# yanyan-li/PlanarSLAM

Measured on NVIDIA H100. Metric: rgbd_frames_per_sec_640x480, higher is better.
Workload: dtype u8/f64

## Files before the change

planarslam_b200/csrc/lsd_kernels.cuh:

```cuda
#pragma once
#include <cuda_runtime.h>

#include <cfloat>
#include <cstdint>

#include "lsd_detsincos.h"
#include "lsd_rectenum.h"
#include "pslam_internal.h"

namespace pslam {

struct LsdGeom {
    int w, h;
    int W, H;
    int refine;
    int seg_cap;
    int cand_cap;
    int rect_enum;
    int min_reg_size;
    double rho, prec, p, log_nt, density_th, log_eps;
    const double* lgamma_tab;
};
#define LSD_LGAMMA_N 8192

#define LSD_ANG_UNDEF 0x7f800000u
#define LSD_ANG_USED 0x80000000u

#define LSD_PI 3.14159265358979323846
#define LSD_DEG2RAD (LSD_PI / 180)
#define LSD_3_2_PI ((3 * LSD_PI) / 2)
#define LSD_2PI (2 * LSD_PI)
#define LSD_LN10 2.30258509299404568402

__device__ __forceinline__ float lsd_fast_atan2_deg(float y, float x) {
    const float p1 = 0.9997878412794807f * (float)(180 / 3.14159265358979323846);
    const float p3 = -0.3258083974640975f * (float)(180 / 3.14159265358979323846);
    const float p5 = 0.1555786518463281f * (float)(180 / 3.14159265358979323846);
    const float p7 = -0.04432655554792128f * (float)(180 / 3.14159265358979323846);
    const float ax = fabsf(x), ay = fabsf(y);
    const bool wide = ax >= ay;
    const float num = wide ? ay : ax, den = __fadd_rn(wide ? ax : ay, (float)DBL_EPSILON);
    const float c = __fdiv_rn(num, den);
    const float c2 = __fmul_rn(c, c);
    float a = __fmul_rn(__fadd_rn(__fmul_rn(__fadd_rn(__fmul_rn(__fadd_rn(__fmul_rn(p7, c2), p5), c2), p3), c2), p1), c);
    if (!wide) a = __fsub_rn(90.f, a);
    if (x < 0) a = __fsub_rn(180.f, a);
    if (y < 0) a = __fsub_rn(360.f, a);
    return a;
}
__device__ __forceinline__ double lsd_angle(int gx, int gy) { return (double)lsd_fast_atan2_deg((float)gx, (float)(-gy)) * LSD_DEG2RAD; }
__device__ __forceinline__ double lsd_norm(int gx, int gy) { return sqrt((double)(gx * gx + gy * gy) / 4.0); }

template <int V>
__device__ __noinline__ void lsd_sincos(double x, double& s, double& c) { lsd_sincos_body(x, s, c); }

#define LSD_TW 64
#define LSD_TH 16
#define LSD_SW 88
#define LSD_SH 28
__global__ void __launch_bounds__(256) k_lsd_blur_scale(LsdGeom g, const uint8_t* __restrict__ gray, const int16_t* __restrict__ ix,
                                                        const int16_t* __restrict__ ax, const int16_t* __restrict__ iy, const int16_t* __restrict__ ay,
                                                        uint8_t* __restrict__ scaled) {
    __shared__ uint8_t s_src[LSD_SH][LSD_SW];
    __shared__ uint16_t s_h[LSD_SH][LSD_SW];
    __shared__ uint8_t s_b[LSD_SH][LSD_SW];
    const int frame = blockIdx.z, X0 = blockIdx.x * LSD_TW, Y0 = blockIdx.y * LSD_TH;
    const int X1 = min(X0 + LSD_TW, g.W) - 1, Y1 = min(Y0 + LSD_TH, g.H) - 1;
    const int bx0 = ix[X0], bx1 = min(ix[X1] + 1, g.w - 1), by0 = iy[Y0], by1 = min(iy[Y1] + 1, g.h - 1);
    const int sx0 = bx0 - 2, sy0 = by0 - 2, sw = bx1 - bx0 + 5, sh = by1 - by0 + 5;
    const uint8_t* src = gray + (size_t)frame * g.w * g.h;
    const int lane = threadIdx.x & 31, wid = threadIdx.x >> 5;
    for (int r = wid; r < sh; r += 8) {
        int y = sy0 + r;
        y = y < 0 ? -y : (y >= g.h ? 2 * (g.h - 1) - y : y);
        const uint8_t* srow = src + (size_t)y * g.w;
        for (int c = lane; c < sw; c += 32) {
            int x = sx0 + c;
            x = x < 0 ? -x : (x >= g.w ? 2 * (g.w - 1) - x : x);
            s_src[r][c] = srow[x];
        }
    }
    __syncthreads();
    const int bw = bx1 - bx0 + 1, bh = by1 - by0 + 1;
    for (int r = wid; r < sh; r += 8)
// ... 51 lines not shown
    const int W4 = g.W >> 2;
    const int xq = blockIdx.x * 64 + (threadIdx.x & 63), y = blockIdx.y * 4 + (threadIdx.x >> 6);
    const bool inside = xq < W4 && y < g.H;
    const uint8_t* s = scaled + (size_t)frame * g.W * g.H;
    uint32_t a_w[4] = {LSD_ANG_UNDEF, LSD_ANG_UNDEF, LSD_ANG_UNDEF, LSD_ANG_UNDEF}, g_w[4] = {0, 0, 0, 0};
    float2 cs[4];
#pragma unroll
    for (int i = 0; i < 4; ++i) cs[i] = make_float2(0.f, 0.f);
    int sq = 0;
    if (inside && y < g.H - 1) {
        const int x = xq * 4;
        const uint32_t* r0 = reinterpret_cast<const uint32_t*>(s + (size_t)y * g.W + x);
        const uint32_t* r1 = reinterpret_cast<const uint32_t*>(s + (size_t)(y + 1) * g.W + x);
        const uint32_t w0 = r0[0], w1 = r1[0];
        const bool more = x + 4 < g.W;
        const uint32_t n0 = more ? (uint32_t)s[(size_t)y * g.W + x + 4] : 0u, n1 = more ? (uint32_t)s[(size_t)(y + 1) * g.W + x + 4] : 0u;
        const uint32_t e0 = __funnelshift_r(w0, n0, 8), e1 = __funnelshift_r(w1, n1, 8);
#pragma unroll
        for (int i = 0; i < 4; ++i) {
            if (x + i >= g.W - 1) continue;
            const int pa = (w0 >> (8 * i)) & 255, pb = (e0 >> (8 * i)) & 255, pc = (w1 >> (8 * i)) & 255, pd = (e1 >> (8 * i)) & 255;
            const int DA = pd - pa, BC = pb - pc;
            const int gx = DA + BC, gy = DA - BC;
            g_w[i] = ((uint32_t)gx & 0xffffu) | ((uint32_t)gy << 16);
            if (lsd_norm(gx, gy) > g.rho) {
                sq = max(sq, gx * gx + gy * gy); a_w[i] = __float_as_uint(lsd_fast_atan2_deg((float)gx, (float)(-gy)));
                cs[i] = __ldg(cs_lut + (gx + 510) * 1021 + (gy + 510));
            }
        }
    }
    if (inside) {
        const size_t o = (size_t)frame * g.W * g.H + (size_t)y * g.W + (size_t)xq * 4;
        *reinterpret_cast<uint4*>(ang + o) = make_uint4(a_w[0], a_w[1], a_w[2], a_w[3]);
        *reinterpret_cast<uint4*>(gxy + o) = make_uint4(g_w[0], g_w[1], g_w[2], g_w[3]);
        float4* co = reinterpret_cast<float4*>(cs_out + o);
        co[0] = make_float4(cs[0].x, cs[0].y, cs[1].x, cs[1].y);
        co[1] = make_float4(cs[2].x, cs[2].y, cs[3].x, cs[3].y);
    }
    for (int o = 16; o; o >>= 1) sq = max(sq, __shfl_xor_sync(0xffffffffu, sq, o));
    if ((threadIdx.x & 31) == 0 && sq > 0) atomicMax(&smax[frame], sq);
}

struct LsdRect { double x1, y1, x2, y2, width, x, y, theta, dx, dy, prec, p; };

#define LSD_RING 64
struct LsdFrame {
    uint32_t* ang;
    const float2* cs; const uint32_t* gxy;
    uint32_t* reg; uint32_t* order;
    int W, H;
};
__device__ __forceinline__ bool lsd_word_used(uint32_t w) { return (w & LSD_ANG_USED) != 0; }
__device__ __forceinline__ bool lsd_word_defined(uint32_t w) { return (w & 0x7fffffffu) < LSD_ANG_UNDEF; }
__device__ __forceinline__ float lsd_word_deg(uint32_t w) { return __uint_as_float(w & 0x7fffffffu); }
__device__ __forceinline__ double lsd_word_angle(uint32_t w) { return (double)lsd_word_deg(w) * LSD_DEG2RAD; }
__device__ __forceinline__ double lsd_pix_norm(const LsdFrame& F, int x, int y) {
    const uint32_t v = __ldg(F.gxy + (size_t)y * F.W + x);
    return lsd_norm((int)(short)(v & 0xffff), (int)(short)(v >> 16));
}

__device__ __forceinline__ bool lsd_aligned_angle(double a, double theta, double prec) {
    double n_theta = theta - a;
    if (n_theta < 0) n_theta = -n_theta;
    if (n_theta > LSD_3_2_PI) {
        n_theta -= LSD_2PI;
        if (n_theta < 0) n_theta = -n_theta;
    }
    return n_theta <= prec;
}

__device__ __forceinline__ double lsd_angle_diff_signed(double a, double b) {
    double diff = a - b;
    while (diff <= -LSD_PI) diff += LSD_2PI;
    while (diff > LSD_PI) diff -= LSD_2PI;
    return diff;
}
__device__ __forceinline__ bool lsd_double_equal(double a, double b) {
    if (a == b) return true;
    const double abs_diff = fabs(a - b), aa = fabs(a), bb = fabs(b);
    double abs_max = (aa > bb) ? aa : bb;
    if (abs_max < DBL_MIN) abs_max = DBL_MIN;
    return (abs_diff / abs_max) <= (100.0 * DBL_EPSILON);
}
__device__ __forceinline__ double lsd_dist_sq(double x1, double y1, double x2, double y2) { return (x2 - x1) * (x2 - x1) + (y2 - y1) * (y2 - y1); }

struct LsdGrown { double angle; int size; };
template <int V>
__device__ __noinline__ LsdGrown lsd_region_grow(uint32_t* ang, const float2* __restrict__ cs, uint32_t* reg, int W, int H, uint32_t seed, double prec) {
    __shared__ uint32_t ring[LSD_RING];
    const int lane = threadIdx.x & 31;
    const unsigned below = (1u << lane) - 1u;
    const int q = lane >> 3, k8 = lane & 7;
    const int kk = k8 + (k8 >= 4);
    const int dyl = kk / 3 - 1, dxl = kk % 3 - 1;
    const int sx = seed & 0xffff, sy = seed >> 16;
    const uint32_t ws = ang[(size_t)sy * W + sx];
    double reg_angle = lsd_word_angle(ws);
    float sumdx = 0.f, sumdy = 0.f;
    if (lane == 0) { reg[0] = seed; ring[0] = seed; ang[(size_t)sy * W + sx] = ws | LSD_ANG_USED; }
    __syncwarp();
    auto probe = [&](int idx, int size, uint32_t& npix, uint32_t& w, float2& csv) {
        const uint32_t pp = size - idx <= LSD_RING ? ring[idx & (LSD_RING - 1)] : reg[idx];
        const int nx = (int)(pp & 0xffff) + dxl, ny = (int)(pp >> 16) + dyl;
        if (nx >= 0 && ny >= 0 && nx < W && ny < H) {
            const size_t o = (size_t)ny * W + nx;
            w = ang[o]; csv = __ldg(cs + o); npix = (uint32_t)nx | ((uint32_t)ny << 16);
        }
    };
    int size = 1, i = 0;
    bool have_next = false;
    uint32_t np_next = 0xffffffffu, w_next = LSD_ANG_UNDEF;
    float2 cs_next = make_float2(0.f, 0.f);
    while (true) {
        const int navail = min(4, size - i);
        uint32_t npix = 0xffffffffu, w = LSD_ANG_UNDEF;
        float2 csv = make_float2(0.f, 0.f);
        if (have_next) { npix = np_next; w = w_next; csv = cs_next; }
        else if (q < navail) probe(i + q, size, npix, w, csv);
        have_next = size - i >= 8;
        np_next = 0xffffffffu; w_next = LSD_ANG_UNDEF; cs_next = make_float2(0.f, 0.f);
        if (have_next) probe(i + 4 + q, size, np_next, w_next, cs_next);
// ... 180 lines not shown
            const bool hole = idx < m && far_point(reg[idx]);
            const unsigned h = __ballot_sync(0xffffffffu, hole);
            if (hole) reg[idx] = reg[size - 1 - (r + __popc(h & below))];
            r += __popc(h);
        }
        __syncwarp();
        size = m;
        if (size < 2) return false;
        lsd_region2rect<V>(F, size, reg_angle, g.prec, g.p, rec);
        density = lsd_density(size, rec);
    }
    return true;
}

__device__ __forceinline__ double lsd_log_gamma1(double x) {
    if (x > 15.0) return 0.918938533204673 + (x - 0.5) * log(x) - x + 0.5 * x * log(x * sinh(1 / x) + 1 / (810.0 * pow(x, 6.0)));
    const double q[7] = {75122.6331530, 80916.6278952, 36308.2951477, 8687.24529705, 1168.92649479, 83.8676043424, 2.50662827511};
    double a = (x + 0.5) * log(x + 5.5) - (x + 5.5);
    double b = 0;
    for (int n = 0; n < 7; ++n) {
        a -= log(x + (double)n);
        b += q[n] * pow(x, (double)n);
    }
    return a + log(b);
}
__device__ __noinline__ double lsd_nfa_scalar(int n, int k, double p, double log_nt, const double* __restrict__ lgamma_tab) {
    if (n == 0 || k == 0) return -log_nt;
    if (n == k) return -log_nt - (double)n * log10(p);
    const double p_term = p / (1 - p);
    double lg0, lg1, lg2;
    if (n + 1 < LSD_LGAMMA_N) { lg0 = __ldg(lgamma_tab + n + 1); lg1 = __ldg(lgamma_tab + k + 1); lg2 = __ldg(lgamma_tab + n - k + 1); }
    else { lg0 = lsd_log_gamma1((double)n + 1); lg1 = lsd_log_gamma1((double)k + 1); lg2 = lsd_log_gamma1((double)(n - k) + 1); }
    const double log1term = lg0 - lg1 - lg2 + (double)k * log(p) + (double)(n - k) * log(1.0 - p);
    double term = exp(log1term);
    if (lsd_double_equal(term, 0)) {
        if (k > n * p) return -log1term / LSD_LN10 - log_nt;
        return -log_nt;
    }
    double bin_tail = term;
    const double tolerance = 0.1;
    for (int i = k + 1; i <= n; ++i) {
        const double bin_term = (double)(n - i + 1) / (double)i;
        const double mult_term = bin_term * p_term;
        term *= mult_term;
        bin_tail += term;
        if (bin_term < 1) {
            const double err = term * ((1 - pow(mult_term, (double)(n - i + 1))) / (1 - mult_term) - 1);
            if (err < tolerance * fabs(-log10(bin_tail) - log_nt) * bin_tail) break;
        }
    }
    return -log10(bin_tail) - log_nt;
}

__device__ __forceinline__ double lsd_inter_low(double x, double x1, double y1, double x2, double y2) {
    if (lsd_double_equal(x1, x2) && y1 < y2) return y1;
    if (lsd_double_equal(x1, x2) && y1 > y2) return y2;
    return y1 + (x - x1) * (y2 - y1) / (x2 - x1);
}
__device__ __forceinline__ double lsd_inter_hi(double x, double x1, double y1, double x2, double y2) {
    if (lsd_double_equal(x1, x2) && y1 < y2) return y2;
    if (lsd_double_equal(x1, x2) && y1 > y2) return y1;
    return y1 + (x - x1) * (y2 - y1) / (x2 - x1);
}

__device__ __forceinline__ void lsd_rect_count(const LsdFrame& F, const LsdGeom& g, const LsdRect& r, int sub, int stride, int& n, int& k) {
    double vx[4], vy[4], rx[4], ry[4];
    vx[0] = r.x1 - r.dy * r.width / 2.0; vy[0] = r.y1 + r.dx * r.width / 2.0;
    vx[1] = r.x2 - r.dy * r.width / 2.0; vy[1] = r.y2 + r.dx * r.width / 2.0;
    vx[2] = r.x2 + r.dy * r.width / 2.0; vy[2] = r.y2 - r.dx * r.width / 2.0;
    vx[3] = r.x1 + r.dy * r.width / 2.0; vy[3] = r.y1 - r.dx * r.width / 2.0;
    int offset;
    if (r.x1 < r.x2 && r.y1 <= r.y2) offset = 0;
    else if (r.x1 >= r.x2 && r.y1 < r.y2) offset = 1;
    else if (r.x1 > r.x2 && r.y1 >= r.y2) offset = 2;
    else offset = 3;
#pragma unroll
    for (int q = 0; q < 4; ++q) { rx[q] = vx[(offset + q) & 3]; ry[q] = vy[(offset + q) & 3]; }
    n = 0; k = 0;
    const int xa = (int)ceil(rx[0]), xb = (int)floor(rx[2]);
    for (int x = xa + sub; x <= xb; x += stride) {
        if (x < 0 || x >= F.W) continue;
        const double ys = (double)x < rx[3] ? lsd_inter_low(x, rx[0], ry[0], rx[3], ry[3]) : lsd_inter_low(x, rx[3], ry[3], rx[2], ry[2]);
        const double ye = (double)x < rx[1] ? lsd_inter_hi(x, rx[0], ry[0], rx[1], ry[1]) : lsd_inter_hi(x, rx[1], ry[1], rx[2], ry[2]);
        for (int y = (int)ceil(ys); (double)y <= ye; ++y) {
            if (y < 0 || y >= F.H) continue;
            ++n;
            const uint32_t wq = __ldg(F.ang + (size_t)y * F.W + x);
            if (lsd_word_defined(wq) && lsd_aligned_angle(lsd_word_angle(wq), r.theta, r.prec)) ++k;
        }
    }
}

__device__ __forceinline__ void lsd_rect_count_cv4(const LsdFrame& F, const LsdGeom& g, const LsdRect& r, int& n, int& k) {
    LsdRowScan S;
    lsd_cv4_setup(r.x1, r.y1, r.x2, r.y2, r.width, r.dx, r.dy, S);
    n = 0; k = 0;
    const int ya = S.y0 < 0 ? 0 : S.y0, yb = S.c2 < F.H - 1 ? S.c2 : F.H - 1;
    for (int y = ya; y <= yb; ++y) {
        int xa, xb;
        lsd_cv4_row(S, y, xa, xb);
        if (xa < 0) xa = 0;
        if (xb > F.W - 1) xb = F.W - 1;
        for (int x = xa; x <= xb; ++x) {
            ++n;
            const uint32_t wq = __ldg(F.ang + (size_t)y * F.W + x);
            if (lsd_word_defined(wq) && lsd_aligned_angle(lsd_word_angle(wq), r.theta, r.prec)) ++k;
        }
    }
}

__device__ __forceinline__ double lsd_rect_nfa_scalar(const LsdFrame& F, const LsdGeom& g, const LsdRect& r) {
    int n, k;
    if (g.rect_enum == 1) lsd_rect_count_cv4(F, g, r, n, k);
    else lsd_rect_count(F, g, r, 0, 1, n, k);
    return lsd_nfa_scalar(n, k, r.p, g.log_nt, g.lgamma_tab);
}
__device__ __forceinline__ void lsd_rect_count_cv4_prec5(const LsdFrame& F, const LsdRect& r, const double prec[5], int& n, int k[5]) {
    LsdRowScan S;
    lsd_cv4_setup(r.x1, r.y1, r.x2, r.y2, r.width, r.dx, r.dy, S);
    n = 0;
#pragma unroll
    for (int j = 0; j < 5; ++j) k[j] = 0;
    const int ya = S.y0 < 0 ? 0 : S.y0, yb = S.c2 < F.H - 1 ? S.c2 : F.H - 1;
    for (int y = ya; y <= yb; ++y) {
        int xa, xb;
        lsd_cv4_row(S, y, xa, xb);
        if (xa < 0) xa = 0;
        if (xb > F.W - 1) xb = F.W - 1;
        for (int x = xa; x <= xb; ++x) {
            ++n;
            const uint32_t wq = __ldg(F.ang + (size_t)y * F.W + x);
            if (!lsd_word_defined(wq)) continue;
            double n_theta = r.theta - lsd_word_angle(wq);
            if (n_theta < 0) n_theta = -n_theta;
            if (n_theta > LSD_3_2_PI) { n_theta -= LSD_2PI; if (n_theta < 0) n_theta = -n_theta; }
#pragma unroll
            for (int j = 0; j < 5; ++j) k[j] += n_theta <= prec[j];
        }
    }
}
__device__ __noinline__ double lsd_rect_improve_rest(const LsdFrame& F, const LsdGeom& g, LsdRect& rec, double log_nfa) {
    const double delta = 0.5, delta_2 = delta / 2.0;
    for (int stage = 0; stage < 5; ++stage) {
        LsdRect r = rec;
        if ((stage == 0 || stage == 4) && g.rect_enum == 1) {
            if (stage == 0 || (r.width - delta) >= 0.5) {
                double pv[5], precv[5];
                int nn, kk[5];
                double pp = r.p;
#pragma unroll
                for (int n = 0; n < 5; ++n) { pp /= 2; pv[n] = pp; precv[n] = pp * LSD_PI; }
                lsd_rect_count_cv4_prec5(F, r, precv, nn, kk);
#pragma unroll
                for (int n = 0; n < 5; ++n) {
                    r.p = pv[n]; r.prec = precv[n];
                    const double v = lsd_nfa_scalar(nn, kk[n], r.p, g.log_nt, g.lgamma_tab);
                    if (v > log_nfa) { log_nfa = v; rec = r; }
                }
            }
            if (stage < 4 && log_nfa > g.log_eps) return log_nfa;
            continue;
        }
        for (int n = 0; n < 5; ++n) {
            if (stage == 0) { r.p /= 2; r.prec = r.p * LSD_PI; }
            else {
                if (!((r.width - delta) >= 0.5)) continue;
                if (stage == 1) r.width -= delta;
                else if (stage == 2) { r.x1 += -r.dy * delta_2; r.y1 += r.dx * delta_2; r.x2 += -r.dy * delta_2; r.y2 += r.dx * delta_2; r.width -= delta; }
                else if (stage == 3) { r.x1 -= -r.dy * delta_2; r.y1 -= r.dx * delta_2; r.x2 -= -r.dy * delta_2; r.y2 -= r.dx * delta_2; r.width -= delta; }
                else { r.p /= 2; r.prec = r.p * LSD_PI; }
            }
            const double v = lsd_rect_nfa_scalar(F, g, r);
            if (v > log_nfa) { log_nfa = v; rec = r; }
        }
        if (stage < 4 && log_nfa > g.log_eps) return log_nfa;
    }
    return log_nfa;
}

#define LSD_ORDER_THREADS 1024
#define LSD_ORDER_SMEM (32 * 1024 * 4)
__device__ __forceinline__ int lsd_order_bin(const uint8_t* __restrict__ s, int W, int x, int y, double rho, double bin_coef) {
    const size_t a = (size_t)y * W + x;
    const int DA = (int)s[a + W + 1] - (int)s[a], BC = (int)s[a + 1] - (int)s[a + W];
    const int gx = DA + BC, gy = DA - BC;
    const double nrm = lsd_norm(gx, gy);
    return nrm > rho ? (int)(nrm * bin_coef) : -1;
}
__global__ void __launch_bounds__(LSD_ORDER_THREADS) k_lsd_order(LsdGeom g, const uint8_t* __restrict__ scaled, const int32_t* __restrict__ smax,
                                                                uint32_t* __restrict__ order_all, int32_t* __restrict__ n_order) {
    extern __shared__ uint32_t s_cnt[];
    __shared__ uint32_t s_tot[1024];
    __shared__ uint32_t s_wsum[32];
    const int frame = blockIdx.x, tid = threadIdx.x, lane = tid & 31, wid = tid >> 5;
    const int sm = smax[frame];
    if (sm <= 0) { if (tid == 0) n_order[frame] = 0; return; }
    const size_t npx = (size_t)g.W * g.H;
    const uint8_t* s = scaled + (size_t)frame * npx;
    uint32_t* order = order_all + (size_t)frame * npx;
    const double max_grad = sqrt((double)sm / 4.0);
    const double bin_coef = (double)(1024 - 1) / max_grad;
    for (int t = tid; t < 32 * 1024; t += LSD_ORDER_THREADS) s_cnt[t] = 0;
    __syncthreads();
    const int Wm = g.W - 1, n_scan = Wm * (g.H - 1);
    const int per = ((n_scan + 31) / 32 + 31) & ~31;
    const int t0 = wid * per, t1 = min(n_scan, t0 + per);
    uint32_t* cnt = s_cnt + wid * 1024;
    for (int base = t0; base < t1; base += 32) {
        const int t = base + lane;
        int bin = -1;
        if (t < t1) { const int y = t / Wm, x = t - y * Wm; bin = lsd_order_bin(s, g.W, x, y, g.rho, bin_coef); }
        const unsigned peers = __match_any_sync(0xffffffffu, bin);
        if (bin >= 0 && lane == __ffs(peers) - 1) cnt[bin] += __popc(peers);
        __syncwarp();
    }
    __syncthreads();
    {
        const int rb = 1023 - tid;
        uint32_t tot = 0;
        for (int w = 0; w < 32; ++w) tot += s_cnt[w * 1024 + rb];
        uint32_t incl = tot;
        for (int o = 1; o < 32; o <<= 1) { const uint32_t v = __shfl_up_sync(0xffffffffu, incl, o); if (lane >= o) incl += v; }
        if (lane == 31) s_wsum[wid] = incl;
        __syncthreads();
        if (wid == 0) {
// ... 37 lines not shown
    LsdFrame F;
    F.ang = ang_all + (size_t)frame * npx; F.cs = cs_all + (size_t)frame * npx; F.gxy = gxy_all + (size_t)frame * npx; F.reg = reg_all + (size_t)frame * npx;
    F.order = const_cast<uint32_t*>(order_all) + (size_t)frame * npx; F.W = g.W; F.H = g.H;
    int count_out = 0;
    const int n_def = smax[frame] > 0 ? n_order[frame] : 0;
    {
        for (int base = 0; base < n_def; base += 32) {
            const uint32_t mypix = base + lane < n_def ? F.order[base + lane] : 0u;
            int last = -1;
            while (true) {
                bool fresh = false;
                if (base + lane < n_def && lane > last) fresh = !lsd_word_used(F.ang[(size_t)(mypix >> 16) * F.W + (mypix & 0xffff)]);
                const unsigned m = __ballot_sync(0xffffffffu, fresh);
                if (!m) break;
                const int j = __ffs(m) - 1;
                last = j;
                const uint32_t seed = __shfl_sync(0xffffffffu, mypix, j);
                const LsdGrown gr = lsd_region_grow<V>(F.ang, F.cs, F.reg, F.W, F.H, seed, g.prec);
                int size = gr.size;
                double reg_angle = gr.angle;
                if (size < g.min_reg_size) continue;
                LsdRect rc;
                lsd_region2rect<V>(F, size, reg_angle, g.prec, g.p, rc);
                if (g.refine > 0 && !lsd_refine<V>(F, g, size, reg_angle, rc)) continue;
                if (count_out < g.cand_cap && lane < 12) {
                    const double v = lane == 0 ? rc.x1 : lane == 1 ? rc.y1 : lane == 2 ? rc.x2 : lane == 3 ? rc.y2 : lane == 4 ? rc.width : lane == 5 ? rc.x :
                                     lane == 6 ? rc.y : lane == 7 ? rc.theta : lane == 8 ? rc.dx : lane == 9 ? rc.dy : lane == 10 ? rc.prec : rc.p;
                    cands[((size_t)frame * g.cand_cap + count_out) * 12 + lane] = v;
                }
                ++count_out;
            }
        }
    }
    if (lane == 0) {
        n_cand[frame] = count_out;
        status[frame] = count_out > g.cand_cap ? 1 : 0;
    }
}

__device__ __forceinline__ void lsd_load_cand(const double* __restrict__ c, LsdRect& rc) {
    rc.x1 = c[0]; rc.y1 = c[1]; rc.x2 = c[2]; rc.y2 = c[3]; rc.width = c[4]; rc.x = c[5]; rc.y = c[6]; rc.theta = c[7]; rc.dx = c[8]; rc.dy = c[9];
    rc.prec = c[10]; rc.p = c[11];
}
__global__ void __launch_bounds__(64) k_lsd_validate(LsdGeom g, const uint32_t* __restrict__ ang_all, const double* __restrict__ cands, const int32_t* __restrict__ n_cand,
                                                     double* __restrict__ cand_nfa, uint32_t* __restrict__ fail_list, int32_t* __restrict__ n_fail) {
    const int frame = blockIdx.y;
    const int ci = blockIdx.x * 64 + threadIdx.x;
    const int n = min(n_cand[frame], g.cand_cap);
    if (ci >= n) return;
    LsdFrame F;
    F.ang = const_cast<uint32_t*>(ang_all) + (size_t)frame * g.W * g.H; F.cs = nullptr; F.gxy = nullptr; F.reg = nullptr; F.order = nullptr; F.W = g.W; F.H = g.H;
    LsdRect rc;
    lsd_load_cand(cands + ((size_t)frame * g.cand_cap + ci) * 12, rc);
    const double log_nfa = lsd_rect_nfa_scalar(F, g, rc);
    cand_nfa[(size_t)frame * g.cand_cap + ci] = log_nfa;
    if (!(log_nfa > g.log_eps)) fail_list[(size_t)frame * g.cand_cap + atomicAdd(&n_fail[frame], 1)] = (uint32_t)ci;
}
__global__ void __launch_bounds__(64) k_lsd_improve(LsdGeom g, const uint32_t* __restrict__ ang_all, double* __restrict__ cands, double* __restrict__ cand_nfa,
                                                    const uint32_t* __restrict__ fail_list, const int32_t* __restrict__ n_fail) {
    const int frame = blockIdx.y;
    const int k = blockIdx.x * 64 + threadIdx.x;
    if (k >= n_fail[frame]) return;
    const int ci = (int)fail_list[(size_t)frame * g.cand_cap + k];
    LsdFrame F;
    F.ang = const_cast<uint32_t*>(ang_all) + (size_t)frame * g.W * g.H; F.cs = nullptr; F.gxy = nullptr; F.reg = nullptr; F.order = nullptr; F.W = g.W; F.H = g.H;
    double* c = cands + ((size_t)frame * g.cand_cap + ci) * 12;
    LsdRect rc;
    lsd_load_cand(c, rc);
    const double log_nfa = lsd_rect_improve_rest(F, g, rc, cand_nfa[(size_t)frame * g.cand_cap + ci]);
    c[0] = rc.x1; c[1] = rc.y1; c[2] = rc.x2; c[3] = rc.y2; c[4] = rc.width; c[11] = rc.p;
    cand_nfa[(size_t)frame * g.cand_cap + ci] = log_nfa;
}

__global__ void __launch_bounds__(256) k_lsd_emit(LsdGeom g, const double* __restrict__ cands, const int32_t* __restrict__ n_cand, const double* __restrict__ cand_nfa,
                                                  float4* __restrict__ segs, double* __restrict__ wpn, int32_t* __restrict__ n_segs, int32_t* __restrict__ status) {
    __shared__ int s_warp[8];
    __shared__ int s_base;
    const int frame = blockIdx.x, tid = threadIdx.x, lane = tid & 31, wid = tid >> 5;
    const int n = min(n_cand[frame], g.cand_cap);
    if (tid == 0) s_base = 0;
    __syncthreads();
    for (int c0 = 0; c0 < n; c0 += 256) {
        const int ci = c0 + tid;
        bool keep = false;
        double nfa = -1;
        if (ci < n) {
            if (g.refine >= 2) { nfa = cand_nfa[(size_t)frame * g.cand_cap + ci]; keep = nfa > g.log_eps; }
            else keep = true;
        }
        const unsigned m = __ballot_sync(0xffffffffu, keep);
        if (lane == 0) s_warp[wid] = __popc(m);
        __syncthreads();
        int off = s_base;
        for (int w = 0; w < wid; ++w) off += s_warp[w];
        const int slot = off + __popc(m & ((1u << lane) - 1u));
        if (keep && slot < g.seg_cap) {
            const double* c = cands + ((size_t)frame * g.cand_cap + ci) * 12;
            double x1 = c[0], y1 = c[1], x2 = c[2], y2 = c[3], width = c[4];
            x1 += 0.5; y1 += 0.5; x2 += 0.5; y2 += 0.5;
            x1 /= 0.8; y1 /= 0.8; x2 /= 0.8; y2 /= 0.8; width /= 0.8;
            segs[(size_t)frame * g.seg_cap + slot] = make_float4((float)x1, (float)y1, (float)x2, (float)y2);
            double* o = wpn + ((size_t)frame * g.seg_cap + slot) * 3;
            o[0] = width; o[1] = c[11]; o[2] = nfa;
        }
        __syncthreads();
        if (tid == 0) { int t = 0; for (int w = 0; w < 8; ++w) t += s_warp[w]; s_base += t; }
        __syncthreads();
// ... 63 lines not shown
```

planarslam_b200/csrc/lsd_pipeline.cu:

```cuda
#include <algorithm>
#include <cfloat>
#include <cmath>
#include <cstring>
#include <cstdlib>
#include <string>

#include "lsd_kernels.cuh"
#include "lbd_kernels.cuh"

namespace pslam {

struct LsdBuffers {
    LsdGeom g;
    int max_batch = 0, last_n = 0, max_lines_cap = 0;
    int16_t *d_ix = nullptr, *d_ax = nullptr, *d_iy = nullptr, *d_ay = nullptr;
    float2* d_lut = nullptr; double* d_lgamma = nullptr;
    uint8_t* d_gray = nullptr;
    uint8_t* d_scaled = nullptr; uint32_t* d_ang = nullptr; float2* d_cs = nullptr; uint32_t* d_gxy = nullptr; int32_t* d_smax = nullptr;
    uint32_t* d_reg = nullptr; uint32_t* d_order = nullptr; int32_t* d_norder = nullptr;
    double* d_cands = nullptr; double* d_cand_nfa = nullptr; int32_t* d_ncand = nullptr;
    uint32_t* d_fail = nullptr; int32_t* d_nfail = nullptr;
    float4* d_segs = nullptr; double* d_wpn = nullptr; int32_t* d_nsegs = nullptr; int32_t* d_status = nullptr;
    LsdKeyLine* d_kl = nullptr; double* d_lf = nullptr; int32_t* d_nkl = nullptr;
    int16_t *d_dx = nullptr, *d_dy = nullptr; float *d_glocal = nullptr, *d_gglobal = nullptr; uint8_t* d_ldesc = nullptr; float* d_lbd72 = nullptr;
    std::vector<int32_t> h_n, h_status;
};

static int lsd_cv_round(double v) { return (int)std::nearbyint(v); }

static float host_fast_atan2_deg(float y, float x) {
    const float p1 = 0.9997878412794807f * (float)(180 / 3.14159265358979323846);
    const float p3 = -0.3258083974640975f * (float)(180 / 3.14159265358979323846);
    const float p5 = 0.1555786518463281f * (float)(180 / 3.14159265358979323846);
    const float p7 = -0.04432655554792128f * (float)(180 / 3.14159265358979323846);
    const float ax = std::fabs(x), ay = std::fabs(y);
    float a, c, c2;
    if (ax >= ay) { c = ay / (ax + (float)DBL_EPSILON); c2 = c * c; a = (((p7 * c2 + p5) * c2 + p3) * c2 + p1) * c; }
    else { c = ax / (ay + (float)DBL_EPSILON); c2 = c * c; a = 90.f - (((p7 * c2 + p5) * c2 + p3) * c2 + p1) * c; }
    if (x < 0) a = 180.f - a;
    if (y < 0) a = 360.f - a;
    return a;
}

static const int LSD_SEG_CAP = 4096;
#define LSD_REGIONS_OCC 24

int lsd_alloc(pslam_ctx* c) {
    if (c->lsd) return PSLAM_OK;
    LsdBuffers* Bp = new LsdBuffers();
    LsdBuffers& B = *Bp;
    LsdGeom& g = B.g;
    g.w = c->cfg.width; g.h = c->cfg.height;
    const double SCALE = 0.8, ANG_TH = 22.5, QUANT = 2.0;
    g.W = lsd_cv_round(g.w * SCALE); g.H = lsd_cv_round(g.h * SCALE);
    if (g.W < 8 || g.H < 8 || g.W > 32767 || g.H > 32767) { delete Bp; return set_error(c, PSLAM_E_INVALID, "image size unsupported by the line-segment detector"); }
    g.refine = 2;
    g.seg_cap = g.cand_cap = std::max(LSD_SEG_CAP, (int)(((long long)LSD_SEG_CAP * g.w * g.h / (640 * 480) + 1023) / 1024 * 1024));
    {
        const char* e = std::getenv("PSLAM_LSD_RECT_ENUM");
        g.rect_enum = (e && (!std::strcmp(e, "published") || !std::strcmp(e, "0"))) ? 0 : 1;
    }
    g.prec = LSD_PI * ANG_TH / 180; g.p = ANG_TH / 180; g.rho = QUANT / std::sin(g.prec);
    g.log_nt = 5 * (std::log10(double(g.W)) + std::log10(double(g.H))) / 2 + std::log10(11.0);
    g.min_reg_size = (int)(size_t)(-g.log_nt / std::log10(g.p));
    g.density_th = 0.7; g.log_eps = 0;
    B.max_batch = c->cfg.max_batch;
    auto coef = [SCALE](int dn, int sn, std::vector<int16_t>& idx, std::vector<int16_t>& a) {
        idx.resize(dn); a.resize(dn);
        const double scale = 1.0 / SCALE;
        for (int d = 0; d < dn; ++d) {
            const double f = (d + 0.5) * scale - 0.5;
            int i = (int)std::floor(f);
            double fr = f - i;
            if (i < 0) { i = 0; fr = 0; }
            if (i >= sn - 1) { i = sn - 1; fr = 0; }
            idx[d] = (int16_t)i; a[d] = (int16_t)std::floor(fr * 256 + 0.5);
        }
    };
    std::vector<int16_t> ix, ax, iy, ay;
    coef(g.W, g.w, ix, ax); coef(g.H, g.h, iy, ay);
    for (int X0 = 0; X0 < g.W; X0 += LSD_TW) {
        const int X1 = std::min(X0 + LSD_TW, g.W) - 1;
        if (std::min(ix[X1] + 1, g.w - 1) - ix[X0] + 5 > LSD_SW) { delete Bp; return set_error(c, PSLAM_E_INVALID, "LSD tile bound (width)"); }
    }
    for (int Y0 = 0; Y0 < g.H; Y0 += LSD_TH) {
        const int Y1 = std::min(Y0 + LSD_TH, g.H) - 1;
        if (std::min(iy[Y1] + 1, g.h - 1) - iy[Y0] + 5 > LSD_SH) { delete Bp; return set_error(c, PSLAM_E_INVALID, "LSD tile bound (height)"); }
    }
    std::vector<float2> lut((size_t)1021 * 1021);
    for (int gx = -510; gx <= 510; ++gx)
        for (int gy = -510; gy <= 510; ++gy) {
            const double ang = (double)host_fast_atan2_deg((float)gx, (float)(-gy)) * LSD_DEG2RAD;
            const float af = (float)ang;
            lut[(size_t)(gx + 510) * 1021 + (gy + 510)] = make_float2(std::cos(af), std::sin(af));
        }
    std::vector<double> lgam(LSD_LGAMMA_N, 0.0);
    for (int i = 1; i < LSD_LGAMMA_N; ++i) {
        const double x = (double)i;
        if (x > 15.0) lgam[i] = 0.918938533204673 + (x - 0.5) * std::log(x) - x + 0.5 * x * std::log(x * std::sinh(1 / x) + 1 / (810.0 * std::pow(x, 6.0)));
        else {
            static const double q[7] = {75122.6331530, 80916.6278952, 36308.2951477, 8687.24529705, 1168.92649479, 83.8676043424, 2.50662827511};
            double a = (x + 0.5) * std::log(x + 5.5) - (x + 5.5), b = 0;
            for (int n = 0; n < 7; ++n) { a -= std::log(x + double(n)); b += q[n] * std::pow(x, double(n)); }
            lgam[i] = a + std::log(b);
        }
    }
    const size_t npx = (size_t)g.W * g.H, nb = (size_t)B.max_batch;
#define LA(ptr, bytes) do { const int rc_ = check_cuda(c, cudaMalloc((void**)&(ptr), (bytes)), "cudaMalloc(lsd)"); if (rc_ != PSLAM_OK) { c->lsd = Bp; lsd_free(c); return rc_; } } while (0)
    LA(B.d_ix, g.W * 2); LA(B.d_ax, g.W * 2); LA(B.d_iy, g.H * 2); LA(B.d_ay, g.H * 2); LA(B.d_lut, lut.size() * sizeof(float2)); LA(B.d_lgamma, LSD_LGAMMA_N * 8);
    LA(B.d_gray, nb * g.w * g.h); LA(B.d_scaled, nb * npx); LA(B.d_ang, nb * npx * 4); LA(B.d_cs, nb * npx * 8); LA(B.d_gxy, nb * npx * 4); LA(B.d_smax, nb * 4);
    LA(B.d_reg, nb * npx * 4); LA(B.d_order, nb * npx * 4); LA(B.d_norder, nb * 4);
    LA(B.d_fail, nb * g.cand_cap * 4); LA(B.d_nfail, nb * 4);
    LA(B.d_cands, nb * g.cand_cap * 12 * 8); LA(B.d_cand_nfa, nb * g.cand_cap * 8); LA(B.d_ncand, nb * 4);
    LA(B.d_segs, nb * g.seg_cap * sizeof(float4)); LA(B.d_wpn, nb * g.seg_cap * 3 * 8); LA(B.d_nsegs, nb * 4); LA(B.d_status, nb * 4);
#undef LA
    cudaStream_t st = c->stream;
    PSLAM_CUDA(c, cudaMemcpyAsync(B.d_ix, ix.data(), g.W * 2, cudaMemcpyHostToDevice, st));
    PSLAM_CUDA(c, cudaMemcpyAsync(B.d_ax, ax.data(), g.W * 2, cudaMemcpyHostToDevice, st));
    PSLAM_CUDA(c, cudaMemcpyAsync(B.d_iy, iy.data(), g.H * 2, cudaMemcpyHostToDevice, st));
    PSLAM_CUDA(c, cudaMemcpyAsync(B.d_ay, ay.data(), g.H * 2, cudaMemcpyHostToDevice, st));
    PSLAM_CUDA(c, cudaMemcpyAsync(B.d_lut, lut.data(), lut.size() * sizeof(float2), cudaMemcpyHostToDevice, st));
    PSLAM_CUDA(c, cudaMemcpyAsync(B.d_lgamma, lgam.data(), LSD_LGAMMA_N * 8, cudaMemcpyHostToDevice, st));
    g.lgamma_tab = B.d_lgamma;
    PSLAM_CUDA(c, cudaStreamSynchronize(st));
    c->lsd = Bp;
    return PSLAM_OK;
}

void lsd_free(pslam_ctx* c) {
    if (!c->lsd) return;
    LsdBuffers& B = *c->lsd;
    for (void* p : {(void*)B.d_ix, (void*)B.d_ax, (void*)B.d_iy, (void*)B.d_ay, (void*)B.d_lut, (void*)B.d_lgamma, (void*)B.d_gray, (void*)B.d_scaled, (void*)B.d_ang, (void*)B.d_cs, (void*)B.d_gxy,
                    (void*)B.d_smax, (void*)B.d_reg, (void*)B.d_order, (void*)B.d_norder, (void*)B.d_segs, (void*)B.d_wpn,
                    (void*)B.d_nsegs, (void*)B.d_status, (void*)B.d_cands, (void*)B.d_cand_nfa, (void*)B.d_ncand, (void*)B.d_fail, (void*)B.d_nfail, (void*)B.d_kl, (void*)B.d_lf, (void*)B.d_nkl, (void*)B.d_dx, (void*)B.d_dy, (void*)B.d_glocal, (void*)B.d_gglobal,
                    (void*)B.d_ldesc, (void*)B.d_lbd72})
        if (p) cudaFree(p);
    delete c->lsd;
    c->lsd = nullptr;
}

int lsd_detect_dev(pslam_ctx* c, const uint8_t* d_gray, int nframes, int refine) {
    int rc = lsd_alloc(c);
    if (rc != PSLAM_OK) return rc;
    LsdBuffers& B = *c->lsd;
    if (nframes < 1 || nframes > B.max_batch) return set_error(c, PSLAM_E_INVALID, "nframes outside [1, max_batch]");
    if (refine < 0 || refine > 2) return set_error(c, PSLAM_E_INVALID, "refine must be 0, 1 or 2");
    LsdGeom g = B.g;
    g.refine = refine;
    cudaStream_t st = c->stream;
    const size_t npx = (size_t)g.W * g.H;
    PSLAM_CUDA(c, cudaMemsetAsync(B.d_smax, 0, (size_t)nframes * 4, st));
    const dim3 gb((g.W + LSD_TW - 1) / LSD_TW, (g.H + LSD_TH - 1) / LSD_TH, nframes);
    PSLAM_LAUNCH(c, "lsd_blur_scale", k_lsd_blur_scale<<<gb, 256, 0, st>>>(g, d_gray, B.d_ix, B.d_ax, B.d_iy, B.d_ay, B.d_scaled));
    if ((g.W & 3) == 0 && !std::getenv("PSLAM_LSD_GRADIENT1")) {
        const dim3 gg4(((g.W >> 2) + 63) / 64, (g.H + 3) / 4, nframes);
        PSLAM_LAUNCH(c, "lsd_gradient", k_lsd_gradient4<<<gg4, 256, 0, st>>>(g, B.d_scaled, B.d_lut, B.d_ang, B.d_cs, B.d_gxy, B.d_smax));
    } else {
        const dim3 gg((g.W + 63) / 64, (g.H + 3) / 4, nframes);
        PSLAM_LAUNCH(c, "lsd_gradient", k_lsd_gradient<<<gg, 256, 0, st>>>(g, B.d_scaled, B.d_lut, B.d_ang, B.d_cs, B.d_gxy, B.d_smax));
    }
    PSLAM_CUDA(c, cudaFuncSetAttribute(k_lsd_order, cudaFuncAttributeMaxDynamicSharedMemorySize, LSD_ORDER_SMEM));
    if ((size_t)B.g.seg_cap * sizeof(float) > 48 * 1024) {
        if ((size_t)B.g.seg_cap * sizeof(float) > 227 * 1024) return set_error(c, PSLAM_E_INVALID, "image too large for the key-line ranking buffer");
        PSLAM_CUDA(c, cudaFuncSetAttribute(k_lsd_keylines, cudaFuncAttributeMaxDynamicSharedMemorySize, (int)(B.g.seg_cap * sizeof(float))));
    }
    PSLAM_LAUNCH(c, "lsd_order", k_lsd_order<<<nframes, LSD_ORDER_THREADS, LSD_ORDER_SMEM, st>>>(g, B.d_scaled, B.d_smax, B.d_order, B.d_norder));
    {
        static const int occ = [] { const char* e = std::getenv("PSLAM_LSD_OCC"); const int v = e ? std::atoi(e) : LSD_REGIONS_OCC; return v == 16 || v == 20 || v == 24 || v == 32 ? v : LSD_REGIONS_OCC; }();
#define LSD_REGIONS_LAUNCH(V) PSLAM_LAUNCH(c, "lsd_regions", k_lsd_regions<V><<<nframes, 32, 0, st>>>(g, nframes, B.d_ang, B.d_cs, B.d_gxy, B.d_smax, B.d_reg, B.d_order, B.d_norder, \
                                                                                                B.d_cands, B.d_ncand, B.d_status))
        if (occ == 16) LSD_REGIONS_LAUNCH(16); else if (occ == 20) LSD_REGIONS_LAUNCH(20); else if (occ == 24) LSD_REGIONS_LAUNCH(24); else LSD_REGIONS_LAUNCH(32);
#undef LSD_REGIONS_LAUNCH
    }
    if (refine >= 2) {
        const dim3 gv((g.cand_cap + 63) / 64, nframes);
        PSLAM_CUDA(c, cudaMemsetAsync(B.d_nfail, 0, (size_t)nframes * 4, st));
        PSLAM_LAUNCH(c, "lsd_validate", k_lsd_validate<<<gv, 64, 0, st>>>(g, B.d_ang, B.d_cands, B.d_ncand, B.d_cand_nfa, B.d_fail, B.d_nfail));
        PSLAM_LAUNCH(c, "lsd_improve", k_lsd_improve<<<gv, 64, 0, st>>>(g, B.d_ang, B.d_cands, B.d_cand_nfa, B.d_fail, B.d_nfail));
    }
    PSLAM_LAUNCH(c, "lsd_emit", k_lsd_emit<<<nframes, 256, 0, st>>>(g, B.d_cands, B.d_ncand, B.d_cand_nfa, B.d_segs, B.d_wpn, B.d_nsegs, B.d_status));
    PSLAM_CUDA(c, cudaGetLastError());
    B.last_n = nframes;
    return PSLAM_OK;
}

// ... 195 lines not shown
```

Baseline: 5981.

## Replace per-pixel angle alignment test with integer ranges and tabulate NFA values

Computes, once per rectangle and precision, up to three ranges of raw angle-word bit patterns that satisfy the double-precision alignment test, found by binary search over the monotone float encoding. Each pixel test becomes three unsigned compares instead of a float-to-double conversion and branches. It also precomputes an NFA table for n up to 512 and p halved up to ten times, so common evaluations become a lookup instead of a series summation. The cost is setup work per rectangle, a larger table built at init, and some risk of edge-case mismatch at range boundaries.

```diff
diff --git a/planarslam_b200/csrc/lsd_alignbounds.h b/planarslam_b200/csrc/lsd_alignbounds.h
--- /dev/null
+++ b/planarslam_b200/csrc/lsd_alignbounds.h
@@ -0,0 +1,89 @@
+#pragma once
+#include <stdint.h>
+#include <string.h>
+
+#include "lsd_rectenum.h"
+
+#define LSD_PI 3.14159265358979323846
+#define LSD_DEG2RAD (LSD_PI / 180)
+#define LSD_3_2_PI ((3 * LSD_PI) / 2)
+#define LSD_2PI (2 * LSD_PI)
+#define LSD_ANG_UNDEF 0x7f800000u
+
+LSD_HD double lsd_word_angle(uint32_t w) {
+    const uint32_t m = w & 0x7fffffffu;
+    float deg;
+    memcpy(&deg, &m, 4);
+    return (double)deg * LSD_DEG2RAD;
+}
+
+LSD_HD bool lsd_aligned_angle(double a, double theta, double prec) {
+    double n_theta = theta - a;
+    if (n_theta < 0) n_theta = -n_theta;
+    if (n_theta > LSD_3_2_PI) {
+        n_theta -= LSD_2PI;
+        if (n_theta < 0) n_theta = -n_theta;
+    }
+    return n_theta <= prec;
+}
+
+struct LsdAlignSet { uint32_t lo[3], len[3]; };
+
+LSD_HD bool lsd_word_aligned(const LsdAlignSet& S, uint32_t w) {
+    const uint32_t m = w & 0x7fffffffu;
+    return (m - S.lo[0] < S.len[0]) | (m - S.lo[1] < S.len[1]) | (m - S.lo[2] < S.len[2]);
+}
+
+LSD_HD uint32_t lsd_ab_guess(double rad) {
+    const double deg = rad * (180 / LSD_PI);
+    if (!(deg > 0)) return 0;
+    if (deg >= 3.0e38) return LSD_ANG_UNDEF - 1;
+    const float f = (float)deg;
+    uint32_t w;
+    memcpy(&w, &f, 4);
+    return w;
+}
+
+template <class Pred>
+LSD_HD uint32_t lsd_ab_first(const Pred& pred, uint32_t guess) {
+    uint32_t lo, hi, step = 1;
+    if (guess >= LSD_ANG_UNDEF) guess = LSD_ANG_UNDEF - 1;
+    if (pred(guess)) {
+        hi = guess;
+        while (true) {
+            if (hi < step) { lo = 0; break; }
+            const uint32_t t = hi - step;
+            if (!pred(t)) { lo = t + 1; break; }
+            hi = t;
+            step *= 2;
+        }
+    } else {
+        lo = guess + 1;
+        while (true) {
+            const uint32_t t = guess + step;
+            if (t >= LSD_ANG_UNDEF) { hi = LSD_ANG_UNDEF; break; }
+            if (pred(t)) { hi = t; break; }
+            lo = t + 1;
+            step *= 2;
+        }
+    }
+    while (lo < hi) {
+        const uint32_t mid = lo + (hi - lo) / 2;
+        if (pred(mid)) hi = mid;
+        else lo = mid + 1;
+    }
+    return lo;
+}
+
+LSD_HD void lsd_align_set(double theta, double prec, LsdAlignSet& S) {
+    const double neg = -prec;
+    auto set = [&S](int i, uint32_t lo, uint32_t end) { S.lo[i] = lo; S.len[i] = end > lo ? end - lo : 0u; };
+    set(0, lsd_ab_first([&](uint32_t w) { return theta - lsd_word_angle(w) <= prec; }, lsd_ab_guess(theta - prec)),
+        lsd_ab_first([&](uint32_t w) { return !(lsd_word_angle(w) - theta <= prec); }, lsd_ab_guess(theta + prec)));
+    set(1, lsd_ab_first([&](uint32_t w) { const double e = theta - lsd_word_angle(w); return e - LSD_2PI <= prec; }, lsd_ab_guess(theta - LSD_2PI - prec)),
+        lsd_ab_first([&](uint32_t w) { const double e = theta - lsd_word_angle(w); return !(e > LSD_3_2_PI && e - LSD_2PI >= neg); },
+                     lsd_ab_guess(theta - LSD_2PI + prec)));
+    set(2, lsd_ab_first([&](uint32_t w) { const double r = lsd_word_angle(w) - theta; return r > LSD_3_2_PI && r - LSD_2PI >= neg; },
+                        lsd_ab_guess(theta + LSD_2PI - prec)),
+        lsd_ab_first([&](uint32_t w) { const double r = lsd_word_angle(w) - theta; return !(r - LSD_2PI <= prec); }, lsd_ab_guess(theta + LSD_2PI + prec)));
+}
diff --git a/planarslam_b200/csrc/lsd_kernels.cuh b/planarslam_b200/csrc/lsd_kernels.cuh
--- a/planarslam_b200/csrc/lsd_kernels.cuh
+++ b/planarslam_b200/csrc/lsd_kernels.cuh
@@ -4,6 +4,7 @@
 #include <cfloat>
 #include <cstdint>
 
+#include "lsd_alignbounds.h"
 #include "lsd_detsincos.h"
 #include "lsd_rectenum.h"
 #include "pslam_internal.h"
@@ -20,16 +21,12 @@
     int min_reg_size;
     double rho, prec, p, log_nt, density_th, log_eps;
     const double* lgamma_tab;
+    const double* nfa_tab;
 };
 #define LSD_LGAMMA_N 8192
 
-#define LSD_ANG_UNDEF 0x7f800000u
 #define LSD_ANG_USED 0x80000000u
 
-#define LSD_PI 3.14159265358979323846
-#define LSD_DEG2RAD (LSD_PI / 180)
-#define LSD_3_2_PI ((3 * LSD_PI) / 2)
-#define LSD_2PI (2 * LSD_PI)
 #define LSD_LN10 2.30258509299404568402
 
 __device__ __forceinline__ float lsd_fast_atan2_deg(float y, float x) {
@@ -187,21 +184,9 @@
 };
 __device__ __forceinline__ bool lsd_word_used(uint32_t w) { return (w & LSD_ANG_USED) != 0; }
 __device__ __forceinline__ bool lsd_word_defined(uint32_t w) { return (w & 0x7fffffffu) < LSD_ANG_UNDEF; }
-__device__ __forceinline__ float lsd_word_deg(uint32_t w) { return __uint_as_float(w & 0x7fffffffu); }
-__device__ __forceinline__ double lsd_word_angle(uint32_t w) { return (double)lsd_word_deg(w) * LSD_DEG2RAD; }
 __device__ __forceinline__ double lsd_pix_norm(const LsdFrame& F, int x, int y) {
     const uint32_t v = __ldg(F.gxy + (size_t)y * F.W + x);
     return lsd_norm((int)(short)(v & 0xffff), (int)(short)(v >> 16));
-}
-
-__device__ __forceinline__ bool lsd_aligned_angle(double a, double theta, double prec) {
-    double n_theta = theta - a;
-    if (n_theta < 0) n_theta = -n_theta;
-    if (n_theta > LSD_3_2_PI) {
-        n_theta -= LSD_2PI;
-        if (n_theta < 0) n_theta = -n_theta;
-    }
-    return n_theta <= prec;
 }
 
 __device__ __forceinline__ double lsd_angle_diff_signed(double a, double b) {
@@ -488,6 +473,28 @@
     return -log10(bin_tail) - log_nt;
 }
 
+#define LSD_NFA_NMAX 512
+#define LSD_NFA_NJ 11
+#define LSD_NFA_TRI ((LSD_NFA_NMAX + 1) * (LSD_NFA_NMAX + 2) / 2)
+__global__ void __launch_bounds__(256) k_lsd_nfa_table(LsdGeom g, double* __restrict__ tab) {
+    const int i = blockIdx.x * 256 + threadIdx.x;
+    if (i >= LSD_NFA_NJ * LSD_NFA_TRI) return;
+    const int j = i / LSD_NFA_TRI, e = i - j * LSD_NFA_TRI;
+    int n = (int)((sqrt(8.0 * e + 1.0) - 1.0) / 2.0);
+    while (n * (n + 1) / 2 > e) --n;
+    while ((n + 1) * (n + 2) / 2 <= e) ++n;
+    double p = g.p;
+    for (int t = 0; t < j; ++t) p /= 2;
+    tab[i] = lsd_nfa_scalar(n, e - n * (n + 1) / 2, p, g.log_nt, g.lgamma_tab);
+}
+__device__ __forceinline__ double lsd_nfa(int n, int k, double p, const LsdGeom& g) {
+    if (n <= LSD_NFA_NMAX) {
+        const int j = ilogb(g.p) - ilogb(p);
+        if (j >= 0 && j < LSD_NFA_NJ && p == ldexp(g.p, -j)) return __ldg(g.nfa_tab + j * LSD_NFA_TRI + n * (n + 1) / 2 + k);
+    }
+    return lsd_nfa_scalar(n, k, p, g.log_nt, g.lgamma_tab);
+}
+
 __device__ __forceinline__ double lsd_inter_low(double x, double x1, double y1, double x2, double y2) {
     if (lsd_double_equal(x1, x2) && y1 < y2) return y1;
     if (lsd_double_equal(x1, x2) && y1 > y2) return y2;
@@ -499,7 +506,7 @@
     return y1 + (x - x1) * (y2 - y1) / (x2 - x1);
 }
 
-__device__ __forceinline__ void lsd_rect_count(const LsdFrame& F, const LsdGeom& g, const LsdRect& r, int sub, int stride, int& n, int& k) {
+__device__ __forceinline__ void lsd_rect_count(const LsdFrame& F, const LsdRect& r, const LsdAlignSet& S, int sub, int stride, int& n, int& k) {
     double vx[4], vy[4], rx[4], ry[4];
     vx[0] = r.x1 - r.dy * r.width / 2.0; vy[0] = r.y1 + r.dx * r.width / 2.0;
     vx[1] = r.x2 - r.dy * r.width / 2.0; vy[1] = r.y2 + r.dx * r.width / 2.0;
@@ -522,12 +529,12 @@
             if (y < 0 || y >= F.H) continue;
             ++n;
             const uint32_t wq = __ldg(F.ang + (size_t)y * F.W + x);
-            if (lsd_word_defined(wq) && lsd_aligned_angle(lsd_word_angle(wq), r.theta, r.prec)) ++k;
-        }
-    }
-}
-
-__device__ __forceinline__ void lsd_rect_count_cv4(const LsdFrame& F, const LsdGeom& g, const LsdRect& r, int& n, int& k) {
+            k += lsd_word_aligned(S, wq);
+        }
+    }
+}
+
+__device__ __forceinline__ void lsd_rect_count_cv4(const LsdFrame& F, const LsdRect& r, const LsdAlignSet& A, int& n, int& k) {
     LsdRowScan S;
     lsd_cv4_setup(r.x1, r.y1, r.x2, r.y2, r.width, r.dx, r.dy, S);
     n = 0; k = 0;
@@ -540,18 +547,18 @@
         for (int x = xa; x <= xb; ++x) {
             ++n;
             const uint32_t wq = __ldg(F.ang + (size_t)y * F.W + x);
-            if (lsd_word_defined(wq) && lsd_aligned_angle(lsd_word_angle(wq), r.theta, r.prec)) ++k;
-        }
-    }
-}
-
-__device__ __forceinline__ double lsd_rect_nfa_scalar(const LsdFrame& F, const LsdGeom& g, const LsdRect& r) {
+            k += lsd_word_aligned(A, wq);
+        }
+    }
+}
+
+__device__ __forceinline__ double lsd_rect_nfa(const LsdFrame& F, const LsdGeom& g, const LsdRect& r, const LsdAlignSet& S) {
     int n, k;
-    if (g.rect_enum == 1) lsd_rect_count_cv4(F, g, r, n, k);
-    else lsd_rect_count(F, g, r, 0, 1, n, k);
-    return lsd_nfa_scalar(n, k, r.p, g.log_nt, g.lgamma_tab);
-}
-__device__ __forceinline__ void lsd_rect_count_cv4_prec5(const LsdFrame& F, const LsdRect& r, const double prec[5], int& n, int k[5]) {
+    if (g.rect_enum == 1) lsd_rect_count_cv4(F, r, S, n, k);
+    else lsd_rect_count(F, r, S, 0, 1, n, k);
+    return lsd_nfa(n, k, r.p, g);
+}
+__device__ __forceinline__ void lsd_rect_count_cv4_prec5(const LsdFrame& F, const LsdRect& r, const LsdAlignSet A[5], int& n, int k[5]) {
     LsdRowScan S;
     lsd_cv4_setup(r.x1, r.y1, r.x2, r.y2, r.width, r.dx, r.dy, S);
     n = 0;
@@ -566,37 +573,36 @@
         for (int x = xa; x <= xb; ++x) {
             ++n;
             const uint32_t wq = __ldg(F.ang + (size_t)y * F.W + x);
-            if (!lsd_word_defined(wq)) continue;
-            double n_theta = r.theta - lsd_word_angle(wq);
-            if (n_theta < 0) n_theta = -n_theta;
-            if (n_theta > LSD_3_2_PI) { n_theta -= LSD_2PI; if (n_theta < 0) n_theta = -n_theta; }
 #pragma unroll
-            for (int j = 0; j < 5; ++j) k[j] += n_theta <= prec[j];
+            for (int j = 0; j < 5; ++j) k[j] += lsd_word_aligned(A[j], wq);
         }
     }
 }
 __device__ __noinline__ double lsd_rect_improve_rest(const LsdFrame& F, const LsdGeom& g, LsdRect& rec, double log_nfa) {
     const double delta = 0.5, delta_2 = delta / 2.0;
+    LsdAlignSet S;
     for (int stage = 0; stage < 5; ++stage) {
         LsdRect r = rec;
         if ((stage == 0 || stage == 4) && g.rect_enum == 1) {
             if (stage == 0 || (r.width - delta) >= 0.5) {
                 double pv[5], precv[5];
+                LsdAlignSet S5[5];
                 int nn, kk[5];
                 double pp = r.p;
 #pragma unroll
-                for (int n = 0; n < 5; ++n) { pp /= 2; pv[n] = pp; precv[n] = pp * LSD_PI; }
-                lsd_rect_count_cv4_prec5(F, r, precv, nn, kk);
+                for (int n = 0; n < 5; ++n) { pp /= 2; pv[n] = pp; precv[n] = pp * LSD_PI; lsd_align_set(r.theta, precv[n], S5[n]); }
+                lsd_rect_count_cv4_prec5(F, r, S5, nn, kk);
 #pragma unroll
                 for (int n = 0; n < 5; ++n) {
                     r.p = pv[n]; r.prec = precv[n];
-                    const double v = lsd_nfa_scalar(nn, kk[n], r.p, g.log_nt, g.lgamma_tab);
+                    const double v = lsd_nfa(nn, kk[n], r.p, g);
                     if (v > log_nfa) { log_nfa = v; rec = r; }
                 }
             }
             if (stage < 4 && log_nfa > g.log_eps) return log_nfa;
             continue;
         }
+        if (stage == 1) lsd_align_set(rec.theta, rec.prec, S);
         for (int n = 0; n < 5; ++n) {
             if (stage == 0) { r.p /= 2; r.prec = r.p * LSD_PI; }
             else {
@@ -606,7 +612,8 @@
                 else if (stage == 3) { r.x1 -= -r.dy * delta_2; r.y1 -= r.dx * delta_2; r.x2 -= -r.dy * delta_2; r.y2 -= r.dx * delta_2; r.width -= delta; }
                 else { r.p /= 2; r.prec = r.p * LSD_PI; }
             }
-            const double v = lsd_rect_nfa_scalar(F, g, r);
+            if (stage == 0 || stage == 4) lsd_align_set(r.theta, r.prec, S);
+            const double v = lsd_rect_nfa(F, g, r, S);
             if (v > log_nfa) { log_nfa = v; rec = r; }
         }
         if (stage < 4 && log_nfa > g.log_eps) return log_nfa;
@@ -750,7 +757,9 @@
     F.ang = const_cast<uint32_t*>(ang_all) + (size_t)frame * g.W * g.H; F.cs = nullptr; F.gxy = nullptr; F.reg = nullptr; F.order = nullptr; F.W = g.W; F.H = g.H;
     LsdRect rc;
     lsd_load_cand(cands + ((size_t)frame * g.cand_cap + ci) * 12, rc);
-    const double log_nfa = lsd_rect_nfa_scalar(F, g, rc);
+    LsdAlignSet S;
+    lsd_align_set(rc.theta, rc.prec, S);
+    const double log_nfa = lsd_rect_nfa(F, g, rc, S);
     cand_nfa[(size_t)frame * g.cand_cap + ci] = log_nfa;
     if (!(log_nfa > g.log_eps)) fail_list[(size_t)frame * g.cand_cap + atomicAdd(&n_fail[frame], 1)] = (uint32_t)ci;
 }
diff --git a/planarslam_b200/csrc/lsd_pipeline.cu b/planarslam_b200/csrc/lsd_pipeline.cu
--- a/planarslam_b200/csrc/lsd_pipeline.cu
+++ b/planarslam_b200/csrc/lsd_pipeline.cu
@@ -14,7 +14,7 @@
     LsdGeom g;
     int max_batch = 0, last_n = 0, max_lines_cap = 0;
     int16_t *d_ix = nullptr, *d_ax = nullptr, *d_iy = nullptr, *d_ay = nullptr;
-    float2* d_lut = nullptr; double* d_lgamma = nullptr;
+    float2* d_lut = nullptr; double* d_lgamma = nullptr; double* d_nfa = nullptr;
     uint8_t* d_gray = nullptr;
     uint8_t* d_scaled = nullptr; uint32_t* d_ang = nullptr; float2* d_cs = nullptr; uint32_t* d_gxy = nullptr; int32_t* d_smax = nullptr;
     uint32_t* d_reg = nullptr; uint32_t* d_order = nullptr; int32_t* d_norder = nullptr;
@@ -108,6 +108,7 @@
     const size_t npx = (size_t)g.W * g.H, nb = (size_t)B.max_batch;
 #define LA(ptr, bytes) do { const int rc_ = check_cuda(c, cudaMalloc((void**)&(ptr), (bytes)), "cudaMalloc(lsd)"); if (rc_ != PSLAM_OK) { c->lsd = Bp; lsd_free(c); return rc_; } } while (0)
     LA(B.d_ix, g.W * 2); LA(B.d_ax, g.W * 2); LA(B.d_iy, g.H * 2); LA(B.d_ay, g.H * 2); LA(B.d_lut, lut.size() * sizeof(float2)); LA(B.d_lgamma, LSD_LGAMMA_N * 8);
+    LA(B.d_nfa, (size_t)LSD_NFA_NJ * LSD_NFA_TRI * 8);
     LA(B.d_gray, nb * g.w * g.h); LA(B.d_scaled, nb * npx); LA(B.d_ang, nb * npx * 4); LA(B.d_cs, nb * npx * 8); LA(B.d_gxy, nb * npx * 4); LA(B.d_smax, nb * 4);
     LA(B.d_reg, nb * npx * 4); LA(B.d_order, nb * npx * 4); LA(B.d_norder, nb * 4);
     LA(B.d_fail, nb * g.cand_cap * 4); LA(B.d_nfail, nb * 4);
@@ -122,6 +123,9 @@
     PSLAM_CUDA(c, cudaMemcpyAsync(B.d_lut, lut.data(), lut.size() * sizeof(float2), cudaMemcpyHostToDevice, st));
     PSLAM_CUDA(c, cudaMemcpyAsync(B.d_lgamma, lgam.data(), LSD_LGAMMA_N * 8, cudaMemcpyHostToDevice, st));
     g.lgamma_tab = B.d_lgamma;
+    g.nfa_tab = B.d_nfa;
+    k_lsd_nfa_table<<<(LSD_NFA_NJ * LSD_NFA_TRI + 255) / 256, 256, 0, st>>>(g, B.d_nfa);
+    PSLAM_CUDA(c, cudaGetLastError());
     PSLAM_CUDA(c, cudaStreamSynchronize(st));
     c->lsd = Bp;
     return PSLAM_OK;
@@ -130,7 +134,7 @@
 void lsd_free(pslam_ctx* c) {
     if (!c->lsd) return;
     LsdBuffers& B = *c->lsd;
-    for (void* p : {(void*)B.d_ix, (void*)B.d_ax, (void*)B.d_iy, (void*)B.d_ay, (void*)B.d_lut, (void*)B.d_lgamma, (void*)B.d_gray, (void*)B.d_scaled, (void*)B.d_ang, (void*)B.d_cs, (void*)B.d_gxy,
+    for (void* p : {(void*)B.d_ix, (void*)B.d_ax, (void*)B.d_iy, (void*)B.d_ay, (void*)B.d_lut, (void*)B.d_lgamma, (void*)B.d_nfa, (void*)B.d_gray, (void*)B.d_scaled, (void*)B.d_ang, (void*)B.d_cs, (void*)B.d_gxy,
                     (void*)B.d_smax, (void*)B.d_reg, (void*)B.d_order, (void*)B.d_norder, (void*)B.d_segs, (void*)B.d_wpn,
                     (void*)B.d_nsegs, (void*)B.d_status, (void*)B.d_cands, (void*)B.d_cand_nfa, (void*)B.d_ncand, (void*)B.d_fail, (void*)B.d_nfail, (void*)B.d_kl, (void*)B.d_lf, (void*)B.d_nkl, (void*)B.d_dx, (void*)B.d_dy, (void*)B.d_glocal, (void*)B.d_gglobal,
                     (void*)B.d_ldesc, (void*)B.d_lbd72})
```

New measurement: 6239, median of 6. 1.04x the previous value.
